# klausondrag/FOSVOS

Hardware: AMD Instinct MI355X
Metric: online fine-tune frames/sec (854x480) (higher is better)
Workload: dtype bf16; 1 GPU; OSVOS_VGG train_online one-shot fine-tune: 1x3x480x854 frame per step, fwd + class-balanced BCE + bwd, fused SGD step every 5 steps (BASELINE.json configs[1]); batch=1, avg_grad_every_n=5, activations=bf16 NHWC, fp32 accumulate, fp32 master weights, parallelism=single GPU

## Files before the change

fosvos_amd/csrc/common.hpp:

```cpp
#pragma once
#include <hip/hip_runtime.h>
#include <stdarg.h>
#include <algorithm>
#include <stdint.h>
#include <stdio.h>
#include <stdlib.h>
#include <string.h>

#include "../../include/fosvos_hip.h"

namespace fosvos {

extern thread_local char g_err[512];

inline int fail(int code, const char *fmt, ...) __attribute__((format(printf, 2, 3)));
inline int fail(int code, const char *fmt, ...) {
    va_list ap;
    va_start(ap, fmt);
    vsnprintf(g_err, sizeof(g_err), fmt, ap);
    va_end(ap);
    return code;
}

#define FOSVOS_HIP_CHECK(expr)                                                                         \
// ... 10 lines not shown
    } while (0)

#define FOSVOS_ENTER(device) FOSVOS_HIP_CHECK(hipSetDevice(device))
extern bool g_prof_on;
void prof_begin(const char *name, hipStream_t st, double flops);
void prof_end();
#define FOSVOS_PROF(name, st, flops)                                        \
    do {                                                                    \
        if (::fosvos::g_prof_on) ::fosvos::prof_begin(name, (hipStream_t)(st), flops); \
    } while (0)
#define FOSVOS_LAUNCH_CHECK()                            \
    do {                                                 \
        if (::fosvos::g_prof_on) ::fosvos::prof_end();   \
        FOSVOS_HIP_CHECK(hipGetLastError());             \
    } while (0)

struct WgradReduceEntry {
    const float *slabs;
    float *dw, *db;
    const float *bias_part;
    int64_t E_real, E_pad;
    int S, S_bias, Co, Cor, accumulate;
    int block_begin, n_blocks;
    int fold_begin, fold_blocks;
};
constexpr int kWgradReduceMax = 20;
struct WgradReduceTable {
    int n;
    WgradReduceEntry e[kWgradReduceMax];
};
int wgrad_impl(const uint16_t *x, const uint16_t *dy, float *dw, float *db, int N, int H, int W, int Ci, int Co,
               int accumulate, void *workspace, size_t workspace_bytes, int device, void *stream,
               WgradReduceTable *reduce, bool alone = false);
int first_wgrad_impl(const float *frame, const uint16_t *dy, float *dw, float *db, int N, int H, int W, int Co,
                     int accumulate, void *workspace, size_t workspace_bytes, int device, void *stream,
                     WgradReduceTable *reduce);
int wgrad_reduce_all(WgradReduceTable *reduce, int device, void *stream);
int wgrad_queue_reduce(const float *slabs, const float *bias_part, float *dw, float *db, int S, int S_bias, int64_t E_real,
                       int64_t E_pad, int Co, int Cor, int accumulate, WgradReduceTable *reduce, int device, void *stream);
struct HeadBwdArgs {
    const float *const *side;
    const int *hs, *ws;
    const float *const *filt, *const *filt1;
    const float *dsn_w, *fuse_w, *d_fused;
    const float *const *d_side_out;
    uint16_t *const *d_side;
    float *d_fuse_w, *d_fuse_b, *d_dsn_w, *d_dsn_b;
// ... 128 lines not shown
```

fosvos_amd/csrc/conv_wgrad.hip:

```cpp
#include <stdlib.h>

#include "common.hpp"

using namespace fosvos;

namespace {
constexpr int TH = 8;
constexpr int TPIX = TH * 16;
constexpr int HALO_W = 18;
constexpr int BCI = 64;

struct WgArgs {
    const uint16_t *x;
    const uint16_t *dy;
    float *slabs;
    float *bias_part;
    int N, H, W, Ci, Cy, Cor;
    int tiles_x, tiles_y, n_tiles, tiles_per_split;
    int lab;
    int S, n_ci, n_co, xcd_order;
};

typedef __attribute__((address_space(3))) s16x4 *lds_s16x4_ptr;

// ... 235 lines not shown
    const int ci = ci0 + wi * 16 + (lane & 15);
#pragma unroll
    for (int u = 0; u < NU; ++u)
#pragma unroll
        for (int r = 0; r < 4; ++r) {
            const int co = co0 + wc * 32 + u * 16 + 4 * g + r;
            if (co >= a.Cor || (a.lab & 1)) continue;
            float *d = slab + ((int64_t)co * a.Ci + ci) * 9;
#pragma unroll
            for (int t = 0; t < 9; ++t) d[t] = acc[t][u][r];
        }
#undef FOSVOS_W2_ROW
#undef FOSVOS_W2_PIECES_OF_ROW
#undef FOSVOS_W2_PIECE_ANY
#undef FOSVOS_W2_TILE_SCALARS
#undef FOSVOS_W2_ADVANCE
#undef FOSVOS_W2_STAGE
#undef FOSVOS_W2_PIECE_X
#undef FOSVOS_W2_PIECE_Y
}
}

constexpr int kFold = 8;

__global__ __launch_bounds__(256) void k_wgrad_fold(const WgradReduceTable t) {
    int e = 0;
    while (e + 1 < t.n && (int)blockIdx.x >= t.e[e + 1].fold_begin) ++e;
    const WgradReduceEntry &q = t.e[e];
    const int local = blockIdx.x - q.fold_begin;
    if (local >= q.fold_blocks) return;
    const int per_group = q.n_blocks;
    const int grp = local / per_group;
    const int64_t i4 = (int64_t)(local - grp * per_group) * 256 + threadIdx.x;
    if (i4 * 4 >= q.E_real) return;
    float *base = const_cast<float *>(q.slabs) + (int64_t)grp * kFold * q.E_pad + i4 * 4;
    const int n = min(kFold, q.S - grp * kFold);
    float4 v[kFold];
#pragma unroll
    for (int j = 0; j < kFold; ++j) v[j] = *reinterpret_cast<const float4 *>(base + (int64_t)min(j, n - 1) * q.E_pad);
    float4 acc = v[0];
#pragma unroll
    for (int j = 1; j < kFold; ++j)
        if (j < n) { acc.x += v[j].x; acc.y += v[j].y; acc.z += v[j].z; acc.w += v[j].w; }
    *reinterpret_cast<float4 *>(base) = acc;
}

__global__ __launch_bounds__(256) void k_wgrad_reduce(const WgradReduceTable t) {
    int e = 0;
    while (e + 1 < t.n && (int)blockIdx.x >= t.e[e + 1].block_begin) ++e;
    const WgradReduceEntry &q = t.e[e];
    const int local = blockIdx.x - q.block_begin;
    const int64_t i4 = (int64_t)local * 256 + threadIdx.x;
    const bool folded = q.fold_blocks > 0;
    const int n_src = folded ? (q.S + kFold - 1) / kFold : q.S;
    const int64_t stride = (folded ? kFold : 1) * q.E_pad;
    if (i4 * 4 < q.E_real) {
        const float *src = q.slabs + i4 * 4;
        float4 acc = make_float4(0.f, 0.f, 0.f, 0.f);
        for (int s0 = 0; s0 < n_src; s0 += 8) {
            float4 v[8];
#pragma unroll
            for (int j = 0; j < 8; ++j) v[j] = *reinterpret_cast<const float4 *>(src + (int64_t)min(s0 + j, n_src - 1) * stride);
#pragma unroll
            for (int j = 0; j < 8; ++j)
                if (s0 + j < n_src) { acc.x += v[j].x; acc.y += v[j].y; acc.z += v[j].z; acc.w += v[j].w; }
        }
        float4 *d = reinterpret_cast<float4 *>(q.dw + i4 * 4);
        if (q.accumulate) {
            const float4 o = *d;
            acc.x += o.x; acc.y += o.y; acc.z += o.z; acc.w += o.w;
        }
        *d = acc;
    }
    if (local == 0 && q.db) {
        __shared__ float s_part[256];
        int Cg = 1;
        while (Cg < q.Co && Cg < 256) Cg <<= 1;
        const int P = 256 / Cg, part = threadIdx.x / Cg, cl = threadIdx.x - part * Cg;
        const int per = (q.S_bias + P - 1) / P, s_lo = part * per, s_hi = min(s_lo + per, q.S_bias);
        for (int co0 = 0; co0 < q.Co; co0 += Cg) {
            const int co = co0 + cl;
            float acc_b = 0.f;
            if (co < q.Co) {
                for (int s0 = s_lo; s0 < s_hi; s0 += 16) {
                    float v[16];
#pragma unroll
                    for (int j = 0; j < 16; ++j) v[j] = q.bias_part[(int64_t)min(s0 + j, s_hi - 1) * q.Cor + co];
#pragma unroll
                    for (int j = 0; j < 16; ++j)
                        if (s0 + j < s_hi) acc_b += v[j];
                }
            }
            if (co0) __syncthreads();
            s_part[threadIdx.x] = acc_b;
            __syncthreads();
// ... 86 lines not shown
extern "C" int fosvos_conv3x3_wgrad_slabs(const uint16_t *x, const uint16_t *dy, int with_bias, int N, int H, int W, int Ci,
                                          int Co, void *workspace, size_t workspace_bytes, int device, void *stream) {
    WgradReduceTable sink;
    sink.n = 0;
    float dummy = 0.f;
    return fosvos::wgrad_impl(x, dy, &dummy, with_bias ? &dummy : nullptr, N, H, W, Ci, Co, 0, workspace, workspace_bytes,
                              device, stream, &sink);
}

int fosvos::wgrad_queue_reduce(const float *slabs, const float *bias_part, float *dw, float *db, int S, int S_bias,
                               int64_t E_real,
                               int64_t E_pad, int Co, int Cor, int accumulate, WgradReduceTable *reduce, int device,
                               void *stream) {
    WgradReduceTable local;
    local.n = 0;
    WgradReduceTable *t = reduce ? reduce : &local;
    FOSVOS_REQUIRE(t->n < kWgradReduceMax, FOSVOS_E_ARG, "wgrad: reduction queue full");
    FOSVOS_REQUIRE(E_real % 4 == 0 && E_pad % 4 == 0, FOSVOS_E_SHAPE, "wgrad: slab size must be a multiple of 4 floats");
    WgradReduceEntry &q = t->e[t->n];
    q.slabs = slabs; q.dw = dw; q.db = db; q.bias_part = db ? bias_part : nullptr;
    q.S = S; q.S_bias = S_bias; q.Co = Co; q.Cor = Cor; q.accumulate = accumulate;
    q.E_real = E_real;
    q.E_pad = E_pad;
    q.n_blocks = (int)cdiv(E_real / 4, 256);
    q.block_begin = t->n ? t->e[t->n - 1].block_begin + t->e[t->n - 1].n_blocks : 0;
    q.fold_blocks = S > kFold ? (int)cdiv(S, kFold) * q.n_blocks : 0;
    q.fold_begin = t->n ? t->e[t->n - 1].fold_begin + t->e[t->n - 1].fold_blocks : 0;
    ++t->n;
    return reduce ? FOSVOS_OK : fosvos::wgrad_reduce_all(t, device, stream);
}

int fosvos::wgrad_reduce_all(WgradReduceTable *reduce, int device, void *stream) {
    FOSVOS_REQUIRE(reduce, FOSVOS_E_ARG, "wgrad_reduce_all: null table");
    if (reduce->n == 0) return FOSVOS_OK;
    FOSVOS_ENTER(device);
    const WgradReduceEntry &last = reduce->e[reduce->n - 1];
    if (last.fold_begin + last.fold_blocks > 0) {
        FOSVOS_PROF("k_wgrad_fold", stream, 0.0);
        hipLaunchKernelGGL(k_wgrad_fold, dim3((unsigned)(last.fold_begin + last.fold_blocks)), dim3(256), 0,
                           (hipStream_t)stream, *reduce);
        FOSVOS_LAUNCH_CHECK();
    }
    FOSVOS_PROF("k_wgrad_reduce", stream, 0.0);
    hipLaunchKernelGGL(k_wgrad_reduce, dim3((unsigned)(last.block_begin + last.n_blocks)), dim3(256), 0, (hipStream_t)stream,
                       *reduce);
    FOSVOS_LAUNCH_CHECK();
    reduce->n = 0;
    return FOSVOS_OK;
}

int fosvos::wgrad_impl(const uint16_t *x, const uint16_t *dy, float *dw, float *db, int N, int H, int W, int Ci, int Co,
                       int accumulate, void *workspace, size_t workspace_bytes, int device, void *stream,
                       WgradReduceTable *reduce, bool alone) {
    FOSVOS_REQUIRE(x && dy && dw && workspace, FOSVOS_E_ARG, "conv3x3_wgrad: null pointer");
    if (int rc = check_shape(N, H, W, Ci, Co, "conv3x3_wgrad")) return rc;
    const Plan p = make_plan(N, H, W, Ci, Co, alone);
    FOSVOS_REQUIRE(workspace_bytes >= p.slab_bytes + p.bias_bytes, FOSVOS_E_WORKSPACE,
                   "conv3x3_wgrad: workspace %zu < %zu", workspace_bytes, p.slab_bytes + p.bias_bytes);
    FOSVOS_ENTER(device);
    hipStream_t st = (hipStream_t)stream;
    WgArgs a;
    a.x = x; a.dy = dy; a.slabs = reinterpret_cast<float *>(workspace);
    a.bias_part = db ? reinterpret_cast<float *>(reinterpret_cast<char *>(workspace) + p.slab_bytes) : nullptr;
    a.N = N; a.H = H; a.W = W; a.Ci = Ci; a.Cy = p.Cy; a.Cor = p.Cor;
    a.tiles_x = p.tiles_x; a.tiles_y = p.tiles_y; a.n_tiles = p.n_tiles; a.tiles_per_split = p.tps;
// ... 37 lines not shown
```

fosvos_amd/csrc/sgd.hip:

```cpp
#include "common.hpp"

using namespace fosvos;

namespace {
__global__ __launch_bounds__(256) void k_sgd(const fosvos_sgd_entry *__restrict__ table, float momentum,
                                              int flags) {
    const bool first_step = flags & FOSVOS_SGD_FIRST_STEP, zero = flags & FOSVOS_SGD_ZERO_GRAD;
    const fosvos_sgd_entry e = table[blockIdx.y];
    if (e.grad == nullptr || e.numel <= 0) return;
    float *__restrict__ p = e.param;
    float *__restrict__ g = const_cast<float *>(e.grad);
    float *__restrict__ m = e.momentum_buf;
    const float lr = e.lr, wd = e.weight_decay;
    const int64_t n = e.numel;
    const bool vec = (((uintptr_t)p | (uintptr_t)g | (uintptr_t)m) & 15) == 0;
    const int64_t n4 = vec ? (n >> 2) : 0;
    for (int64_t i = blockIdx.x * (int64_t)blockDim.x + threadIdx.x; i < n4; i += (int64_t)gridDim.x * blockDim.x) {
        float4 pv = reinterpret_cast<float4 *>(p)[i];
        const float4 gv = reinterpret_cast<const float4 *>(g)[i];
        float4 mv = first_step ? make_float4(0, 0, 0, 0) : reinterpret_cast<float4 *>(m)[i];
        float pp[4] = {pv.x, pv.y, pv.z, pv.w}, gg[4] = {gv.x, gv.y, gv.z, gv.w}, mm[4] = {mv.x, mv.y, mv.z, mv.w};
#pragma unroll
        for (int j = 0; j < 4; ++j) {
            const float d = wd != 0.f ? gg[j] + wd * pp[j] : gg[j];
            mm[j] = first_step ? d : momentum * mm[j] + d;
            pp[j] = pp[j] - lr * mm[j];
        }
        reinterpret_cast<float4 *>(p)[i] = make_float4(pp[0], pp[1], pp[2], pp[3]);
        reinterpret_cast<float4 *>(m)[i] = make_float4(mm[0], mm[1], mm[2], mm[3]);
        if (zero) reinterpret_cast<float4 *>(g)[i] = make_float4(0.f, 0.f, 0.f, 0.f);
    }
    for (int64_t i = n4 * 4 + blockIdx.x * (int64_t)blockDim.x + threadIdx.x; i < n;
         i += (int64_t)gridDim.x * blockDim.x) {
        const float d = wd != 0.f ? g[i] + wd * p[i] : g[i];
        const float mm = first_step ? d : momentum * m[i] + d;
        m[i] = mm;
        p[i] = p[i] - lr * mm;
        if (zero) g[i] = 0.f;
    }
}
}

extern "C" int fosvos_sgd_momentum_step(const fosvos_sgd_entry *table, int n_tensors, int64_t max_numel, float momentum,
                                        int first_step, int device, void *stream) {
    FOSVOS_REQUIRE(table, FOSVOS_E_ARG, "sgd_momentum_step: null table");
    FOSVOS_REQUIRE(n_tensors > 0 && n_tensors <= 65535 && max_numel > 0, FOSVOS_E_SHAPE,
                   "sgd_momentum_step: n_tensors=%d max_numel=%lld", n_tensors, (long long)max_numel);
    FOSVOS_ENTER(device);
    int64_t gx = cdiv(max_numel, 256 * 4);
    if (gx > 512) gx = 512;
    FOSVOS_PROF("k_sgd", stream, 0.0);
    hipLaunchKernelGGL(k_sgd, dim3((unsigned)gx, (unsigned)n_tensors), dim3(256), 0, (hipStream_t)stream, table,
                       momentum, first_step);
    FOSVOS_LAUNCH_CHECK();
    return FOSVOS_OK;
}
```

fosvos_amd/fosvos_hip/__init__.py:

```python
from __future__ import annotations

import ctypes
import os
import threading
from ctypes import POINTER, c_char_p, c_float, c_int, c_int64, c_size_t, c_uint, c_void_p

_HERE = os.path.dirname(os.path.abspath(__file__))
PKG_ROOT = os.path.dirname(_HERE)
LIB_PATH = os.environ.get("FOSVOS_HIP_LIB") or os.path.join(PKG_ROOT, "lib", "libfosvos_hip.so")
HEADER_PATH = os.path.join(os.path.dirname(PKG_ROOT), "include", "fosvos_hip.h")

ABI_VERSION = 27
CONV_RELU = 1
CONV_OUT_F32 = 2


class FosvosHipError(RuntimeError):
    pass


class SgdEntry(ctypes.Structure):
    _fields_ = [("param", c_void_p), ("grad", c_void_p), ("momentum_buf", c_void_p), ("numel", c_int64),
                ("lr", c_float), ("weight_decay", c_float)]


_P4 = c_void_p * 4
_I4 = c_int * 4
_P13 = c_void_p * 13


class VggWeights(ctypes.Structure):
    _fields_ = [("conv_w", _P13), ("conv_b", _P13), ("conv_wf", _P13), ("conv_wd", _P13),
                ("side_b", _P4), ("side_wf", _P4), ("side_wd", _P4), ("filt", _P4), ("filt1", _P4),
                ("dsn_w", c_void_p), ("dsn_b", c_void_p), ("fuse_w", c_void_p), ("fuse_b", c_void_p),
                ("filt_uniform", c_int)]


class VggGrads(ctypes.Structure):
    _fields_ = [("conv_w", _P13), ("conv_b", _P13), ("side_w", _P4), ("side_b", _P4),
                ("dsn_w", c_void_p), ("dsn_b", c_void_p), ("fuse_w", c_void_p), ("fuse_b", c_void_p),
                ("accumulate", c_int), ("defer_join", c_int), ("bucket_events", c_int), ("last_pass_of_cycle", c_int)]

_Z4 = c_size_t * 4
_Z13 = c_size_t * 13


# ... 88 lines not shown
    "fosvos_maxpool2x2_ceil_bwd": (c_int, [c_void_p, c_void_p, c_void_p, c_int, c_int, c_int, c_int, c_int, c_int,
                                           c_void_p]),
    "fosvos_head_fwd": (c_int, [POINTER(c_void_p), POINTER(c_int), POINTER(c_int), POINTER(c_void_p),
                                POINTER(c_void_p), c_void_p, c_void_p, c_void_p, c_void_p, c_void_p,
                                POINTER(c_void_p), c_int, c_int, c_int, c_int, c_int, c_void_p]),
    "fosvos_head_bwd": (c_int, [POINTER(c_void_p), POINTER(c_int), POINTER(c_int), POINTER(c_void_p),
                                POINTER(c_void_p), c_void_p, c_void_p, c_void_p, POINTER(c_void_p),
                                POINTER(c_void_p), c_void_p, c_void_p, c_void_p, c_void_p, c_int, c_int, c_int, c_int,
                                c_void_p, c_size_t, c_int, c_void_p]),
    "fosvos_head_bwd_workspace_bytes": (c_size_t, [c_int, c_int, c_int]),
    "fosvos_cbce_loss": (c_int, [c_void_p, c_void_p, c_int64, c_int, c_float, c_void_p, c_void_p, c_void_p, c_size_t,
                                 c_int, c_void_p]),
    "fosvos_cbce_workspace_bytes": (c_size_t, [c_int64]),
    "fosvos_cbce_loss_frames": (c_int, [c_void_p, c_void_p, c_int64, c_int, c_int, c_float, c_void_p, c_void_p, c_void_p,
                                        c_size_t, c_int, c_void_p]),
    "fosvos_cbce_loss_frames_parts": (c_int, [c_void_p, c_void_p, c_int64, c_int, c_int, c_float, c_void_p, c_void_p,
                                              c_void_p, c_size_t, c_int, c_int, c_void_p]),
    "fosvos_cbce_multi_workspace_bytes": (c_size_t, [c_int64, c_int, c_int]),
    "fosvos_cbce_loss_frames_multi": (c_int, [POINTER(c_void_p), c_void_p, c_int64, c_int, c_int, c_int, POINTER(c_float),
                                              c_void_p, POINTER(c_void_p), c_void_p, c_size_t, c_int, c_int, c_void_p]),
    "fosvos_cbce_loss_batch_counts": (c_int, [c_void_p, c_void_p, c_int64, c_int, c_float, c_void_p, c_void_p, c_void_p,
                                              c_void_p, c_size_t, c_int, c_void_p]),
    "fosvos_sgd_momentum_step": (c_int, [c_void_p, c_int, c_int64, c_float, c_int, c_int, c_void_p]),
    "fosvos_conv3x3_s2_fwd": (c_int, [c_void_p, c_void_p, c_void_p, c_void_p, c_int, c_int, c_int, c_int, c_int, c_uint,
                                      c_void_p, c_size_t, c_int, c_void_p]),
    "fosvos_conv3x3_fwd_add": (c_int, [c_void_p, c_void_p, c_void_p, c_void_p, c_void_p, c_int, c_int, c_int, c_int, c_int,
                                       c_uint, c_void_p, c_size_t, c_int, c_void_p]),
    "fosvos_fold_conv_bn": (c_int, [c_void_p, c_int, c_int, c_int, c_void_p, c_void_p, c_void_p, c_void_p, c_void_p,
                                    c_float, c_void_p, c_void_p, c_int, c_void_p]),
    "fosvos_conv2d_packed_dwords": (c_size_t, [c_int, c_int, c_int]),
    "fosvos_conv2d_bias_elems": (c_size_t, [c_int]),
    "fosvos_pack_conv2d_bn": (c_int, [c_void_p, c_int, c_int, c_int, c_void_p, c_void_p, c_void_p, c_void_p, c_void_p,
                                      c_float, c_void_p, c_void_p, c_int, c_void_p]),
    "fosvos_conv2d_plan": (c_int, [c_int, c_int, c_int, c_int, c_int, c_int, c_int, POINTER(Conv2dPlanInfo)]),
    "fosvos_conv2d_fwd": (c_int, [c_void_p, c_void_p, c_void_p, c_void_p, c_void_p, c_int, c_int, c_int, c_int, c_int,
                                  c_int, c_int, c_uint, c_int, c_void_p]),
    "fosvos_conv7x7_packed_elems": (c_size_t, [c_int]),
    "fosvos_pack_conv7x7_bn": (c_int, [c_void_p, c_int, c_void_p, c_void_p, c_void_p, c_void_p, c_float, c_void_p,
                                       c_void_p, c_int, c_void_p]),
    "fosvos_conv7x7s2_first_fwd": (c_int, [c_void_p, c_void_p, c_void_p, c_void_p, c_int, c_int, c_int, c_int, c_uint,
                                           c_int, c_void_p]),
    "fosvos_conv7x7s2_pool_first_fwd": (c_int, [c_void_p, c_void_p, c_void_p, c_void_p, c_int, c_int, c_int, c_int, c_int,
                                                c_void_p]),
    "fosvos_maxpool3x3s2_fwd": (c_int, [c_void_p, c_void_p, c_int, c_int, c_int, c_int, c_int, c_void_p]),
    "fosvos_deconv_head_fwd": (c_int, [POINTER(c_void_p), POINTER(c_int), POINTER(c_int), POINTER(c_int),
                                       POINTER(c_void_p), POINTER(c_void_p), c_void_p, c_void_p, c_void_p, c_void_p,
# ... 120 lines not shown
```

fosvos_amd/fosvos_hip/engine.py:

```python
from __future__ import annotations

import ctypes
import time
from dataclasses import dataclass
from typing import Dict, List, Optional, Sequence, Tuple

import torch

from . import Context, VggGrads, VggWeights, check, lib, ops, ptr_array4
from .options import EngineOptions, native_loop_from_env

STAGE_CHANNELS = ((64, 64), (128, 128), (256, 256, 256), (512, 512, 512), (512, 512, 512))
STAGE_IN = (3, 64, 128, 256, 512)
SIDE_CH = 16


def conv_module_index(stage: int, k: int) -> int:
    return 2 * k + (0 if stage == 0 else 1)


def param_names() -> List[str]:
    names = [f"upscale.{i}.weight" for i in range(4)] + [f"upscale_.{i}.weight" for i in range(4)]
    for s, chans in enumerate(STAGE_CHANNELS):
        for j in range(len(chans)):
            m = conv_module_index(s, j)
            names += [f"stages.{s}.{m}.weight", f"stages.{s}.{m}.bias"]
    for i in range(4):
        names += [f"side_prep.{i}.weight", f"side_prep.{i}.bias"]
    for i in range(4):
        names += [f"score_dsn.{i}.weight", f"score_dsn.{i}.bias"]
    names += ["fuse.weight", "fuse.bias"]
    return names


PARAM_NAMES = param_names()
PARAM_INDEX = {n: i for i, n in enumerate(PARAM_NAMES)}


@dataclass(slots=True)
class PassFlags:

    defer_wgrad_join: bool = False
    forward_one_stream: bool = False
    publish_grad_buckets: bool = False
    overwrite_grads: bool = False
    last_pass_of_cycle: bool = False


class PackedWeights:

    def __init__(self, options: Optional[EngineOptions] = None) -> None:
        self.options = options if options is not None else EngineOptions.from_env()
        self.flags = PassFlags()
        self._cache: Dict[str, Tuple[object, object, object]] = {}
        self._uniform: Dict[str, bool] = {}
        self.arenas = ArenaPool()

    @staticmethod
    def _key(t: torch.Tensor) -> Tuple[int, int]:
        return (t.data_ptr(), t._version)

    def invalidate(self) -> None:
        self._cache.clear()
        self._uniform.clear()

    def small(self, name: str, parts: Sequence[torch.Tensor]) -> torch.Tensor:
        key = tuple(self._key(t) for t in parts)
        hit = self._cache.get(name)
        if hit is not None and hit[0] == key:
            return hit[1]
        cat = torch.cat([t.detach().reshape(-1) for t in parts]).contiguous()
        self._cache[name] = (key, cat, tuple(t.untyped_storage() for t in parts))
        return cat

    def conv(self, name: str, w: torch.Tensor):
        key = self._key(w)
        hit = self._cache.get(name)
        if hit is not None and hit[0] == key:
            return hit[1]
        packed = ops.pack_conv3x3_weights(w.detach(), True, True)
        self._cache[name] = (key, packed, w.untyped_storage())
        return packed

    def conv_many(self, named: Sequence[Tuple[str, torch.Tensor]]):
        stale = []
        for name, w in named:
            hit = self._cache.get(name)
            if hit is None or hit[0] != self._key(w):
                stale.append((name, w))
        if stale:
            packed = ops.pack_conv3x3_weights_multi([w.detach() for _, w in stale])
            for (name, w), pk in zip(stale, packed):
                self._cache[name] = (self._key(w), pk, w.untyped_storage())
        return [self._cache[name][1] for name, _ in named]

    def deconv_diag(self, name: str, w: torch.Tensor) -> torch.Tensor:
        key = self._key(w)
        hit = self._cache.get(name)
        if hit is not None and hit[0] == key:
            return hit[1]
        wd = w.detach()
        c = wd.shape[0]
        idx = torch.arange(c, device=wd.device)
        diag = wd[idx, idx]
        if c > 1:
            off = torch.count_nonzero(wd) - torch.count_nonzero(diag)
            if int(off) != 0:
                raise NotImplementedError(
                    f"{name}: transposed-conv weight has off-diagonal (cross-channel) entries; the HIP head "
                    f"implements the per-channel (diagonal) form the reference initialises and freezes")
        diag = diag.permute(1, 2, 0).contiguous()
        self._cache[name] = (key, diag, w.untyped_storage())
        self._uniform[name] = bool((diag == diag[..., :1]).all().item())
        return diag

    def head_uniform_mask(self, P: Dict[str, torch.Tensor]) -> int:
# ... 485 lines not shown
```

fosvos_amd/fosvos_hip/sgd.py:

```python
from __future__ import annotations

import ctypes

import torch
from torch import optim

from . import SgdEntry, check, lib


class FusedSGD(optim.SGD):
    def __init__(self, params, lr=1e-3, momentum=0, dampening=0, weight_decay=0, nesterov=False, **kw):
        if dampening != 0 or nesterov:
            raise NotImplementedError("FusedSGD implements the reference recipe: dampening=0, nesterov=False")
        kw.pop("foreach", None)
        kw.pop("fused", None)
        super().__init__(params, lr=lr, momentum=momentum, dampening=dampening, weight_decay=weight_decay,
                         nesterov=nesterov, **kw)
        self._tables = {}

    @torch.no_grad()
    def step(self, closure=None, only=None, tag="all", zero_grad=False):
        only_ids = None if only is None else {id(p) for p in only}
        loss = None
        if closure is not None:
            with torch.enable_grad():
                loss = closure()
        entries = []
        momentum = None
        device = None
        max_numel = 0
        keep_alive = []
        zero_after = []
        updated = []
        for group in self.param_groups:
            if group.get("dampening", 0) != 0 or group.get("nesterov", False):
                raise NotImplementedError("FusedSGD: dampening/nesterov are not implemented")
            m = float(group["momentum"])
            if momentum is None:
                momentum = m
            elif m != momentum:
                raise NotImplementedError("FusedSGD: one momentum value for all groups (as in the reference recipe)")
            for p in group["params"]:
                if p.grad is None or (only_ids is not None and id(p) not in only_ids):
                    continue
                if not p.is_cuda:
                    raise RuntimeError("FusedSGD: parameters must live on the GPU (no CPU fallback)")
                if p.dtype != torch.float32 or not p.is_contiguous():
                    raise TypeError("FusedSGD: fp32 contiguous parameters only")
                g = p.grad
                if g.dtype != torch.float32 or not g.is_contiguous():
                    g = g.contiguous().float()
                    keep_alive.append(g)
                    if zero_grad:
                        zero_after.append(p.grad)
                st = self.state[p]
                buf = st.get("momentum_buffer")
                if buf is None:
                    buf = torch.zeros_like(p, memory_format=torch.contiguous_format)
                    st["momentum_buffer"] = buf
                device = p.device
                entries.append((p.data_ptr(), g.data_ptr(), buf.data_ptr(), p.numel(), float(group["lr"]),
                                float(group["weight_decay"])))
                if float(group["lr"]) != 0.0:
                    updated.append(p)
                max_numel = max(max_numel, p.numel())
        if not entries:
            return loss
        n = len(entries)
        nbytes = n * ctypes.sizeof(SgdEntry)
        tab = self._tables.setdefault(tag, {"entries": None, "host": None, "dev": None, "event": None})
        if entries != tab["entries"]:
            if tab["host"] is None or tab["host"].numel() < nbytes:
                tab["host"] = torch.empty(max(nbytes, 4096), dtype=torch.uint8).pin_memory()
                tab["dev"] = torch.empty(max(nbytes, 4096), dtype=torch.uint8, device=device)
            if tab["event"] is not None:
                tab["event"].synchronize()
            arr = (SgdEntry * n).from_address(tab["host"].data_ptr())
            for i, e in enumerate(entries):
                arr[i].param, arr[i].grad, arr[i].momentum_buf, arr[i].numel, arr[i].lr, arr[i].weight_decay = e
            tab["dev"][:nbytes].copy_(tab["host"][:nbytes], non_blocking=True)
            tab["event"] = torch.cuda.Event()
            tab["event"].record()
            tab["entries"] = entries
        idx = device.index if device.index is not None else torch.cuda.current_device()
        check(lib().fosvos_sgd_momentum_step(tab["dev"].data_ptr(), n, max_numel, momentum, 2 if zero_grad else 0, idx,
                                             torch.cuda.current_stream(idx).cuda_stream), "sgd_momentum_step")
        for p in updated:
            torch.autograd.graph.increment_version(p)
        for g in zero_after:
            g.zero_()
        del keep_alive
        return loss
```

include/fosvos_hip.h:

```cpp
#ifndef FOSVOS_HIP_H
#define FOSVOS_HIP_H

#include <stddef.h>
#include <stdint.h>

#ifdef __cplusplus
extern "C" {
#endif

#define FOSVOS_ABI_VERSION 27

#define FOSVOS_OK 0
#define FOSVOS_E_SHAPE (-1)
#define FOSVOS_E_ARG (-2)
#define FOSVOS_E_WORKSPACE (-3)
#define FOSVOS_E_HIP (-4)

#define FOSVOS_CONV_RELU 1u
#define FOSVOS_CONV_OUT_F32 2u
#define FOSVOS_CONV_FP32_MATH 4u

int fosvos_abi_version(void);

typedef struct fosvos_profile_record {
    char name[96];
    int launches;
    double ms;
    double flops;
} fosvos_profile_record;
int fosvos_profile_start(int device, int max_launches);
int fosvos_profile_stop(int device, fosvos_profile_record *out, int capacity, int *n_out);
const char *fosvos_last_error(void);
const char *fosvos_build_arch(void);
// ... 111 lines not shown
                                  int size_average, float grad_scale, float *loss_out, float *grad, void *workspace,
                                  size_t workspace_bytes, int parts, int device, void *stream);
#define FOSVOS_CBCE_MAX_MAPS 8
size_t fosvos_cbce_multi_workspace_bytes(int64_t frame_numel, int n_frames, int n_maps);
int fosvos_cbce_loss_frames_multi(const float *const *logits, const float *label, int64_t frame_numel, int n_frames,
                                  int n_maps, int size_average, const float *map_scale, float *loss_out, float *const *grad,
                                  void *workspace, size_t workspace_bytes, int parts, int device, void *stream);
int fosvos_cbce_loss_batch_counts(const float *logits, const float *label, int64_t numel, int size_average,
                                  float grad_scale, const double *batch_counts, float *loss_out, float *grad,
                                  void *workspace, size_t workspace_bytes, int device, void *stream);

#define FOSVOS_SGD_FIRST_STEP 1
#define FOSVOS_SGD_ZERO_GRAD 2
typedef struct fosvos_sgd_entry {
    float *param;
    const float *grad;
    float *momentum_buf;
    int64_t numel;
    float lr;
    float weight_decay;
} fosvos_sgd_entry;
int fosvos_sgd_momentum_step(const fosvos_sgd_entry *table, int n_tensors, int64_t max_numel, float momentum,
                             int first_step, int device, void *stream);

int fosvos_augment_sample(const uint8_t *frame, const uint8_t *mask, int H, int W, int flip, const int32_t *col_taps,
                          const float *col_w, const int32_t *row_taps, const float *row_w, const int32_t *col_near,
                          const int32_t *row_near, int OH, int OW, const float *img_lut, const float *gt_lut, float *image,
                          float *gt, int device, void *stream);

int fosvos_prob_bytes(const float *logits, int N, int H, int W, float *minmax, uint8_t *out, int device, void *stream);
size_t fosvos_jf_workspace_bytes(int N, int H, int W);
int fosvos_jf_counts(const float *logits, const uint8_t *gt, int N, int H, int W, int radius, int32_t *counts,
                     void *workspace, size_t workspace_bytes, int device, void *stream);

size_t fosvos_png_capacity_bytes(int N, int H, int W);
size_t fosvos_png_workspace_bytes(int N, int H, int W);
int fosvos_png_encode(const uint8_t *bytes, int N, int H, int W, uint8_t *out, size_t capacity, int32_t *lengths,
                      void *workspace, size_t workspace_bytes, int device, void *stream);

size_t fosvos_png_workspace_bytes_mode(int N, int H, int W, int huffman);
int fosvos_png_encode_mode(const uint8_t *bytes, int N, int H, int W, int huffman, uint8_t *out, size_t capacity,
                           int32_t *lengths, void *workspace, size_t workspace_bytes, int device, void *stream);

size_t fosvos_jpeg_capacity_bytes(int N, int H, int W, int components);
size_t fosvos_jpeg_workspace_bytes(int N, int H, int W, int components);
int fosvos_jpeg_encode(const uint8_t *frames, int N, int H, int W, int components, int quality, uint8_t *out,
// ... 122 lines not shown
```

Baseline: 1265 frames/s.

## Fuse conv weight repacking into SGD step and merge wgrad fold into reduce

```diff
diff --git a/fosvos_amd/csrc/common.hpp b/fosvos_amd/csrc/common.hpp
--- a/fosvos_amd/csrc/common.hpp
+++ b/fosvos_amd/csrc/common.hpp
@@ -56,7 +56,7 @@
     int64_t E_real, E_pad;
     int S, S_bias, Co, Cor, accumulate;
     int block_begin, n_blocks;
-    int fold_begin, fold_blocks;
+    int cols;
 };
 constexpr int kWgradReduceMax = 20;
 struct WgradReduceTable {
diff --git a/fosvos_amd/csrc/conv_wgrad.hip b/fosvos_amd/csrc/conv_wgrad.hip
--- a/fosvos_amd/csrc/conv_wgrad.hip
+++ b/fosvos_amd/csrc/conv_wgrad.hip
@@ -281,55 +281,75 @@
 }
 
 constexpr int kFold = 8;
-
-__global__ __launch_bounds__(256) void k_wgrad_fold(const WgradReduceTable t) {
-    int e = 0;
-    while (e + 1 < t.n && (int)blockIdx.x >= t.e[e + 1].fold_begin) ++e;
-    const WgradReduceEntry &q = t.e[e];
-    const int local = blockIdx.x - q.fold_begin;
-    if (local >= q.fold_blocks) return;
-    const int per_group = q.n_blocks;
-    const int grp = local / per_group;
-    const int64_t i4 = (int64_t)(local - grp * per_group) * 256 + threadIdx.x;
-    if (i4 * 4 >= q.E_real) return;
-    float *base = const_cast<float *>(q.slabs) + (int64_t)grp * kFold * q.E_pad + i4 * 4;
-    const int n = min(kFold, q.S - grp * kFold);
-    float4 v[kFold];
-#pragma unroll
-    for (int j = 0; j < kFold; ++j) v[j] = *reinterpret_cast<const float4 *>(base + (int64_t)min(j, n - 1) * q.E_pad);
-    float4 acc = v[0];
-#pragma unroll
-    for (int j = 1; j < kFold; ++j)
-        if (j < n) { acc.x += v[j].x; acc.y += v[j].y; acc.z += v[j].z; acc.w += v[j].w; }
-    *reinterpret_cast<float4 *>(base) = acc;
+constexpr int kReduceDirect = 256;
+
+int reduce_cols(int S) {
+    if (S <= kFold) return kReduceDirect;
+    const int G = (S + kFold - 1) / kFold;
+    int gt = 4;
+    while (gt < G && gt < 32) gt <<= 1;
+    return 256 / gt;
 }
 
 __global__ __launch_bounds__(256) void k_wgrad_reduce(const WgradReduceTable t) {
+    __shared__ float s_grp[256 * 4];
     int e = 0;
     while (e + 1 < t.n && (int)blockIdx.x >= t.e[e + 1].block_begin) ++e;
     const WgradReduceEntry &q = t.e[e];
     const int local = blockIdx.x - q.block_begin;
-    const int64_t i4 = (int64_t)local * 256 + threadIdx.x;
-    const bool folded = q.fold_blocks > 0;
-    const int n_src = folded ? (q.S + kFold - 1) / kFold : q.S;
-    const int64_t stride = (folded ? kFold : 1) * q.E_pad;
-    if (i4 * 4 < q.E_real) {
-        const float *src = q.slabs + i4 * 4;
-        float4 acc = make_float4(0.f, 0.f, 0.f, 0.f);
-        for (int s0 = 0; s0 < n_src; s0 += 8) {
-            float4 v[8];
-#pragma unroll
-            for (int j = 0; j < 8; ++j) v[j] = *reinterpret_cast<const float4 *>(src + (int64_t)min(s0 + j, n_src - 1) * stride);
-#pragma unroll
-            for (int j = 0; j < 8; ++j)
-                if (s0 + j < n_src) { acc.x += v[j].x; acc.y += v[j].y; acc.z += v[j].z; acc.w += v[j].w; }
-        }
-        float4 *d = reinterpret_cast<float4 *>(q.dw + i4 * 4);
-        if (q.accumulate) {
-            const float4 o = *d;
-            acc.x += o.x; acc.y += o.y; acc.z += o.z; acc.w += o.w;
-        }
-        *d = acc;
+    if (q.cols == kReduceDirect) {
+        const int64_t i4 = (int64_t)local * 256 + threadIdx.x;
+        if (i4 * 4 < q.E_real) {
+            const float *src = q.slabs + i4 * 4;
+            float4 acc = make_float4(0.f, 0.f, 0.f, 0.f);
+            for (int s0 = 0; s0 < q.S; s0 += 8) {
+                float4 v[8];
+#pragma unroll
+                for (int j = 0; j < 8; ++j) v[j] = *reinterpret_cast<const float4 *>(src + (int64_t)min(s0 + j, q.S - 1) * q.E_pad);
+#pragma unroll
+                for (int j = 0; j < 8; ++j)
+                    if (s0 + j < q.S) { acc.x += v[j].x; acc.y += v[j].y; acc.z += v[j].z; acc.w += v[j].w; }
+            }
+            float4 *d = reinterpret_cast<float4 *>(q.dw + i4 * 4);
+            if (q.accumulate) {
+                const float4 o = *d;
+                acc.x += o.x; acc.y += o.y; acc.z += o.z; acc.w += o.w;
+            }
+            *d = acc;
+        }
+    } else {
+        const int C = q.cols, GT = 256 / C;
+        const int col = threadIdx.x & (C - 1), gt = threadIdx.x / C;
+        const int64_t i4 = (int64_t)local * C + col;
+        const bool live = i4 * 4 < q.E_real;
+        const int G = (q.S + kFold - 1) / kFold;
+        float tot = 0.f;
+        for (int g0 = 0; g0 < G; g0 += GT) {
+            const int grp = g0 + gt;
+            if (live && grp < G) {
+                const float *base = q.slabs + (int64_t)grp * kFold * q.E_pad + i4 * 4;
+                const int n = min(kFold, q.S - grp * kFold);
+                float4 v[kFold];
+#pragma unroll
+                for (int j = 0; j < kFold; ++j) v[j] = *reinterpret_cast<const float4 *>(base + (int64_t)min(j, n - 1) * q.E_pad);
+                float4 acc = v[0];
+#pragma unroll
+                for (int j = 1; j < kFold; ++j)
+                    if (j < n) { acc.x += v[j].x; acc.y += v[j].y; acc.z += v[j].z; acc.w += v[j].w; }
+                *reinterpret_cast<float4 *>(s_grp + (gt * C + col) * 4) = acc;
+            }
+            __syncthreads();
+            if ((int)threadIdx.x < 4 * C) {
+                const int ng = min(GT, G - g0);
+                for (int j = 0; j < ng; ++j) tot += s_grp[j * C * 4 + threadIdx.x];
+            }
+            __syncthreads();
+        }
+        const int64_t f = (int64_t)local * C * 4 + threadIdx.x;
+        if ((int)threadIdx.x < 4 * C && f < q.E_real) {
+            if (q.accumulate) tot += q.dw[f];
+            q.dw[f] = tot;
+        }
     }
     if (local == 0 && q.db) {
         __shared__ float s_part[256];
@@ -462,10 +482,9 @@
     q.S = S; q.S_bias = S_bias; q.Co = Co; q.Cor = Cor; q.accumulate = accumulate;
     q.E_real = E_real;
     q.E_pad = E_pad;
-    q.n_blocks = (int)cdiv(E_real / 4, 256);
+    q.cols = reduce_cols(S);
+    q.n_blocks = (int)cdiv(E_real / 4, q.cols);
     q.block_begin = t->n ? t->e[t->n - 1].block_begin + t->e[t->n - 1].n_blocks : 0;
-    q.fold_blocks = S > kFold ? (int)cdiv(S, kFold) * q.n_blocks : 0;
-    q.fold_begin = t->n ? t->e[t->n - 1].fold_begin + t->e[t->n - 1].fold_blocks : 0;
     ++t->n;
     return reduce ? FOSVOS_OK : fosvos::wgrad_reduce_all(t, device, stream);
 }
@@ -475,12 +494,6 @@
     if (reduce->n == 0) return FOSVOS_OK;
     FOSVOS_ENTER(device);
     const WgradReduceEntry &last = reduce->e[reduce->n - 1];
-    if (last.fold_begin + last.fold_blocks > 0) {
-        FOSVOS_PROF("k_wgrad_fold", stream, 0.0);
-        hipLaunchKernelGGL(k_wgrad_fold, dim3((unsigned)(last.fold_begin + last.fold_blocks)), dim3(256), 0,
-                           (hipStream_t)stream, *reduce);
-        FOSVOS_LAUNCH_CHECK();
-    }
     FOSVOS_PROF("k_wgrad_reduce", stream, 0.0);
     hipLaunchKernelGGL(k_wgrad_reduce, dim3((unsigned)(last.block_begin + last.n_blocks)), dim3(256), 0, (hipStream_t)stream,
                        *reduce);
diff --git a/fosvos_amd/csrc/sgd.hip b/fosvos_amd/csrc/sgd.hip
--- a/fosvos_amd/csrc/sgd.hip
+++ b/fosvos_amd/csrc/sgd.hip
@@ -3,11 +3,14 @@
 using namespace fosvos;
 
 namespace {
-__global__ __launch_bounds__(256) void k_sgd(const fosvos_sgd_entry *__restrict__ table, float momentum,
-                                              int flags) {
-    const bool first_step = flags & FOSVOS_SGD_FIRST_STEP, zero = flags & FOSVOS_SGD_ZERO_GRAD;
-    const fosvos_sgd_entry e = table[blockIdx.y];
-    if (e.grad == nullptr || e.numel <= 0) return;
+__device__ __forceinline__ void sgd_update(float &p, float g, float &m, float lr, float wd, float momentum, bool first_step) {
+    const float d = wd != 0.f ? g + wd * p : g;
+    m = first_step ? d : momentum * m + d;
+    p = p - lr * m;
+}
+
+template <class E>
+__device__ __forceinline__ void sgd_elementwise(const E &e, float momentum, bool first_step, bool zero) {
     float *__restrict__ p = e.param;
     float *__restrict__ g = const_cast<float *>(e.grad);
     float *__restrict__ m = e.momentum_buf;
@@ -21,22 +24,107 @@
         float4 mv = first_step ? make_float4(0, 0, 0, 0) : reinterpret_cast<float4 *>(m)[i];
         float pp[4] = {pv.x, pv.y, pv.z, pv.w}, gg[4] = {gv.x, gv.y, gv.z, gv.w}, mm[4] = {mv.x, mv.y, mv.z, mv.w};
 #pragma unroll
-        for (int j = 0; j < 4; ++j) {
-            const float d = wd != 0.f ? gg[j] + wd * pp[j] : gg[j];
-            mm[j] = first_step ? d : momentum * mm[j] + d;
-            pp[j] = pp[j] - lr * mm[j];
-        }
+        for (int j = 0; j < 4; ++j) sgd_update(pp[j], gg[j], mm[j], lr, wd, momentum, first_step);
         reinterpret_cast<float4 *>(p)[i] = make_float4(pp[0], pp[1], pp[2], pp[3]);
         reinterpret_cast<float4 *>(m)[i] = make_float4(mm[0], mm[1], mm[2], mm[3]);
         if (zero) reinterpret_cast<float4 *>(g)[i] = make_float4(0.f, 0.f, 0.f, 0.f);
     }
     for (int64_t i = n4 * 4 + blockIdx.x * (int64_t)blockDim.x + threadIdx.x; i < n;
          i += (int64_t)gridDim.x * blockDim.x) {
-        const float d = wd != 0.f ? g[i] + wd * p[i] : g[i];
-        const float mm = first_step ? d : momentum * m[i] + d;
+        float pp = p[i], mm = first_step ? 0.f : m[i];
+        sgd_update(pp, g[i], mm, lr, wd, momentum, first_step);
         m[i] = mm;
-        p[i] = p[i] - lr * mm;
+        p[i] = pp;
         if (zero) g[i] = 0.f;
+    }
+}
+
+__global__ __launch_bounds__(256) void k_sgd(const fosvos_sgd_entry *__restrict__ table, float momentum,
+                                              int flags) {
+    const fosvos_sgd_entry e = table[blockIdx.y];
+    if (e.grad == nullptr || e.numel <= 0) return;
+    sgd_elementwise(e, momentum, flags & FOSVOS_SGD_FIRST_STEP, flags & FOSVOS_SGD_ZERO_GRAD);
+}
+
+__global__ __launch_bounds__(256) void k_sgd_pack(const fosvos_sgd_pack_entry *__restrict__ table, float momentum, int flags,
+                                                   int co_t) {
+    __shared__ float tile[32][289];
+    const bool first_step = flags & FOSVOS_SGD_FIRST_STEP, zero = flags & FOSVOS_SGD_ZERO_GRAD;
+    const fosvos_sgd_pack_entry e = table[blockIdx.y];
+    if (e.grad == nullptr || e.numel <= 0) return;
+    if (e.w_fwd == nullptr && e.w_dgrad == nullptr) {
+        sgd_elementwise(e, momentum, first_step, zero);
+        return;
+    }
+    float *__restrict__ p = e.param;
+    float *__restrict__ g = const_cast<float *>(e.grad);
+    float *__restrict__ m = e.momentum_buf;
+    const float lr = e.lr, wd = e.weight_decay;
+    const int Co = e.Co, Ci = e.Ci, nkb = Ci / 32;
+    const int n_tiles = (Co + 31) / 32 * 32 / co_t * nkb;
+    const int co_pad = (Co + 15) / 16 * 16, ci_pad = (Ci + 15) / 16 * 16;
+    const bool vec = (((uintptr_t)p | (uintptr_t)g | (uintptr_t)m) & 15) == 0;
+    for (int t = blockIdx.x; t < n_tiles; t += gridDim.x) {
+        const int cb = t / nkb, kb = t - cb * nkb;
+        const int co0 = cb * co_t, ci0 = kb * 32;
+        if (vec) {
+            for (int i = threadIdx.x; i < co_t * 72; i += 256) {
+                const int r = i / 72, c = (i - r * 72) * 4;
+                float pp[4] = {0.f, 0.f, 0.f, 0.f};
+                if (co0 + r < Co) {
+                    const int64_t at = ((int64_t)(co0 + r) * Ci + ci0) * 9 + c;
+                    const float4 pv = *reinterpret_cast<const float4 *>(p + at), gv = *reinterpret_cast<const float4 *>(g + at);
+                    const float4 mv = first_step ? make_float4(0, 0, 0, 0) : *reinterpret_cast<const float4 *>(m + at);
+                    float gg[4] = {gv.x, gv.y, gv.z, gv.w}, mm[4] = {mv.x, mv.y, mv.z, mv.w};
+                    pp[0] = pv.x; pp[1] = pv.y; pp[2] = pv.z; pp[3] = pv.w;
+#pragma unroll
+                    for (int j = 0; j < 4; ++j) sgd_update(pp[j], gg[j], mm[j], lr, wd, momentum, first_step);
+                    *reinterpret_cast<float4 *>(p + at) = make_float4(pp[0], pp[1], pp[2], pp[3]);
+                    *reinterpret_cast<float4 *>(m + at) = make_float4(mm[0], mm[1], mm[2], mm[3]);
+                    if (zero) *reinterpret_cast<float4 *>(g + at) = make_float4(0.f, 0.f, 0.f, 0.f);
+                }
+                tile[r][c] = pp[0]; tile[r][c + 1] = pp[1]; tile[r][c + 2] = pp[2]; tile[r][c + 3] = pp[3];
+            }
+        } else {
+            for (int i = threadIdx.x; i < co_t * 288; i += 256) {
+                const int r = i / 288, c = i - r * 288;
+                float pp = 0.f;
+                if (co0 + r < Co) {
+                    const int64_t at = ((int64_t)(co0 + r) * Ci + ci0) * 9 + c;
+                    float mm = first_step ? 0.f : m[at];
+                    pp = p[at];
+                    sgd_update(pp, g[at], mm, lr, wd, momentum, first_step);
+                    p[at] = pp;
+                    m[at] = mm;
+                    if (zero) g[at] = 0.f;
+                }
+                tile[r][c] = pp;
+            }
+        }
+        __syncthreads();
+        if (e.w_fwd) {
+            for (int q = threadIdx.x; q < 9 * 4 * co_t; q += 256) {
+                const int l = q % co_t, kc = (q / co_t) & 3, tap = q / (4 * co_t);
+                if (co0 + l >= co_pad) continue;
+                float f[8];
+#pragma unroll
+                for (int j = 0; j < 8; ++j) f[j] = tile[l][(kc * 8 + j) * 9 + tap];
+                *reinterpret_cast<uint4 *>(e.w_fwd + ((((int64_t)kb * 9 + tap) * 4 + kc) * co_pad + co0 + l) * 8) = pack8(f);
+            }
+        }
+        if (e.w_dgrad) {
+            const int n_kc = co_t / 8;
+            for (int q = threadIdx.x; q < 9 * n_kc * 32; q += 256) {
+                const int l = q & 31, kc = (q >> 5) % n_kc, tap = (q >> 5) / n_kc;
+                float f[8];
+#pragma unroll
+                for (int j = 0; j < 8; ++j) f[j] = tile[kc * 8 + j][l * 9 + tap];
+                const int co = co0 + kc * 8;
+                *reinterpret_cast<uint4 *>(e.w_dgrad + ((((int64_t)(co >> 5) * 9 + (8 - tap)) * 4 + ((co >> 3) & 3)) * ci_pad + ci0 + l) * 8) =
+                    pack8(f);
+            }
+        }
+        __syncthreads();
     }
 }
 }
@@ -55,3 +143,22 @@
     FOSVOS_LAUNCH_CHECK();
     return FOSVOS_OK;
 }
+
+extern "C" int fosvos_sgd_momentum_step_pack(const fosvos_sgd_pack_entry *table, int n_tensors, int64_t max_numel,
+                                             int pack_tiles, int max_pack_tiles, float momentum, int flags, int device,
+                                             void *stream) {
+    FOSVOS_REQUIRE(table, FOSVOS_E_ARG, "sgd_momentum_step_pack: null table");
+    FOSVOS_REQUIRE(n_tensors > 0 && n_tensors <= 65535 && max_numel > 0, FOSVOS_E_SHAPE,
+                   "sgd_momentum_step_pack: n_tensors=%d max_numel=%lld", n_tensors, (long long)max_numel);
+    FOSVOS_REQUIRE(pack_tiles >= 0 && max_pack_tiles >= 0 && max_pack_tiles <= pack_tiles, FOSVOS_E_ARG,
+                   "sgd_momentum_step_pack: pack_tiles=%d max_pack_tiles=%d", pack_tiles, max_pack_tiles);
+    FOSVOS_ENTER(device);
+    const int co_t = pack_tiles < 256 ? 8 : 32;
+    int64_t gx = std::max<int64_t>(cdiv(max_numel, 256 * 4), (int64_t)max_pack_tiles * (32 / co_t));
+    if (gx > 512) gx = 512;
+    FOSVOS_PROF(pack_tiles ? "k_sgd_pack" : "k_sgd", stream, 0.0);
+    hipLaunchKernelGGL(k_sgd_pack, dim3((unsigned)gx, (unsigned)n_tensors), dim3(256), 0, (hipStream_t)stream, table, momentum,
+                       flags, co_t);
+    FOSVOS_LAUNCH_CHECK();
+    return FOSVOS_OK;
+}
diff --git a/fosvos_amd/fosvos_hip/__init__.py b/fosvos_amd/fosvos_hip/__init__.py
--- a/fosvos_amd/fosvos_hip/__init__.py
+++ b/fosvos_amd/fosvos_hip/__init__.py
@@ -10,7 +10,7 @@
 LIB_PATH = os.environ.get("FOSVOS_HIP_LIB") or os.path.join(PKG_ROOT, "lib", "libfosvos_hip.so")
 HEADER_PATH = os.path.join(os.path.dirname(PKG_ROOT), "include", "fosvos_hip.h")
 
-ABI_VERSION = 27
+ABI_VERSION = 28
 CONV_RELU = 1
 CONV_OUT_F32 = 2
 
@@ -22,6 +22,12 @@
 class SgdEntry(ctypes.Structure):
     _fields_ = [("param", c_void_p), ("grad", c_void_p), ("momentum_buf", c_void_p), ("numel", c_int64),
                 ("lr", c_float), ("weight_decay", c_float)]
+
+
+class SgdPackEntry(ctypes.Structure):
+    _fields_ = [("param", c_void_p), ("grad", c_void_p), ("momentum_buf", c_void_p), ("numel", c_int64),
+                ("lr", c_float), ("weight_decay", c_float), ("w_fwd", c_void_p), ("w_dgrad", c_void_p), ("Co", c_int),
+                ("Ci", c_int)]
 
 
 _P4 = c_void_p * 4
@@ -156,6 +162,7 @@
     "fosvos_cbce_loss_batch_counts": (c_int, [c_void_p, c_void_p, c_int64, c_int, c_float, c_void_p, c_void_p, c_void_p,
                                               c_void_p, c_size_t, c_int, c_void_p]),
     "fosvos_sgd_momentum_step": (c_int, [c_void_p, c_int, c_int64, c_float, c_int, c_int, c_void_p]),
+    "fosvos_sgd_momentum_step_pack": (c_int, [c_void_p, c_int, c_int64, c_int, c_int, c_float, c_int, c_int, c_void_p]),
     "fosvos_conv3x3_s2_fwd": (c_int, [c_void_p, c_void_p, c_void_p, c_void_p, c_int, c_int, c_int, c_int, c_int, c_uint,
                                       c_void_p, c_size_t, c_int, c_void_p]),
     "fosvos_conv3x3_fwd_add": (c_int, [c_void_p, c_void_p, c_void_p, c_void_p, c_void_p, c_int, c_int, c_int, c_int, c_int,
diff --git a/fosvos_amd/fosvos_hip/engine.py b/fosvos_amd/fosvos_hip/engine.py
--- a/fosvos_amd/fosvos_hip/engine.py
+++ b/fosvos_amd/fosvos_hip/engine.py
@@ -2,6 +2,7 @@
 
 import ctypes
 import time
+import weakref
 from dataclasses import dataclass
 from typing import Dict, List, Optional, Sequence, Tuple
 
@@ -47,6 +48,17 @@
     last_pass_of_cycle: bool = False
 
 
+_LIVE_CACHES: "weakref.WeakSet[PackedWeights]" = weakref.WeakSet()
+
+
+def step_image_slot(w: torch.Tensor):
+    for packs in _LIVE_CACHES:
+        hit = packs.step_images(w)
+        if hit is not None:
+            return packs, hit[0], hit[1]
+    return None
+
+
 class PackedWeights:
 
     def __init__(self, options: Optional[EngineOptions] = None) -> None:
@@ -54,7 +66,9 @@
         self.flags = PassFlags()
         self._cache: Dict[str, Tuple[object, object, object]] = {}
         self._uniform: Dict[str, bool] = {}
+        self._conv_by_ptr: Dict[int, str] = {}
         self.arenas = ArenaPool()
+        _LIVE_CACHES.add(self)
 
     @staticmethod
     def _key(t: torch.Tensor) -> Tuple[int, int]:
@@ -63,6 +77,23 @@
     def invalidate(self) -> None:
         self._cache.clear()
         self._uniform.clear()
+        self._conv_by_ptr.clear()
+
+    def _put_conv(self, name: str, w: torch.Tensor, packed) -> None:
+        self._cache[name] = (self._key(w), packed, w.untyped_storage())
+        self._conv_by_ptr[w.data_ptr()] = name
+
+    def step_images(self, w: torch.Tensor):
+        name = self._conv_by_ptr.get(w.data_ptr())
+        hit = self._cache.get(name) if name is not None else None
+        if hit is None or hit[0][0] != w.data_ptr() or not isinstance(hit[1], tuple) or hit[1][0] is None or hit[1][1] is None:
+            return None
+        return name, hit[1]
+
+    def adopt(self, name: str, w: torch.Tensor, images) -> None:
+        hit = self._cache.get(name)
+        if hit is not None and hit[1] is images:
+            self._cache[name] = (self._key(w), images, hit[2])
 
     def small(self, name: str, parts: Sequence[torch.Tensor]) -> torch.Tensor:
         key = tuple(self._key(t) for t in parts)
@@ -79,7 +110,7 @@
         if hit is not None and hit[0] == key:
             return hit[1]
         packed = ops.pack_conv3x3_weights(w.detach(), True, True)
-        self._cache[name] = (key, packed, w.untyped_storage())
+        self._put_conv(name, w, packed)
         return packed
 
     def conv_many(self, named: Sequence[Tuple[str, torch.Tensor]]):
@@ -91,7 +122,7 @@
         if stale:
             packed = ops.pack_conv3x3_weights_multi([w.detach() for _, w in stale])
             for (name, w), pk in zip(stale, packed):
-                self._cache[name] = (self._key(w), pk, w.untyped_storage())
+                self._put_conv(name, w, pk)
         return [self._cache[name][1] for name, _ in named]
 
     def deconv_diag(self, name: str, w: torch.Tensor) -> torch.Tensor:
diff --git a/fosvos_amd/fosvos_hip/sgd.py b/fosvos_amd/fosvos_hip/sgd.py
--- a/fosvos_amd/fosvos_hip/sgd.py
+++ b/fosvos_amd/fosvos_hip/sgd.py
@@ -5,7 +5,7 @@
 import torch
 from torch import optim
 
-from . import SgdEntry, check, lib
+from . import SgdPackEntry, check, lib
 
 
 class FusedSGD(optim.SGD):
@@ -20,6 +20,7 @@
 
     @torch.no_grad()
     def step(self, closure=None, only=None, tag="all", zero_grad=False):
+        from . import engine
         only_ids = None if only is None else {id(p) for p in only}
         loss = None
         if closure is not None:
@@ -32,6 +33,8 @@
         keep_alive = []
         zero_after = []
         updated = []
+        adopted = []
+        pack_tiles = max_pack_tiles = 0
         for group in self.param_groups:
             if group.get("dampening", 0) != 0 or group.get("nesterov", False):
                 raise NotImplementedError("FusedSGD: dampening/nesterov are not implemented")
@@ -59,15 +62,30 @@
                     buf = torch.zeros_like(p, memory_format=torch.contiguous_format)
                     st["momentum_buffer"] = buf
                 device = p.device
+                wf = wd = co = ci = 0
+                if p.dim() == 4 and p.shape[2:] == (3, 3) and p.shape[1] % 32 == 0:
+                    slot = engine.step_image_slot(p)
+                    co, ci = int(p.shape[0]), int(p.shape[1])
+                    if slot is not None and (slot[2][0].numel() != ci * 9 * ((co + 15) // 16 * 16)
+                                             or slot[2][1].numel() != (co + 31) // 32 * 32 * 9 * ((ci + 15) // 16 * 16)):
+                        slot = None
+                    if slot is None:
+                        co = ci = 0
+                    else:
+                        wf, wd = slot[2][0].data_ptr(), slot[2][1].data_ptr()
+                        tiles = (co + 31) // 32 * (ci // 32)
+                        pack_tiles += tiles
+                        max_pack_tiles = max(max_pack_tiles, tiles)
+                        adopted.append((slot[0], slot[1], slot[2], p))
                 entries.append((p.data_ptr(), g.data_ptr(), buf.data_ptr(), p.numel(), float(group["lr"]),
-                                float(group["weight_decay"])))
+                                float(group["weight_decay"]), wf, wd, co, ci))
                 if float(group["lr"]) != 0.0:
                     updated.append(p)
                 max_numel = max(max_numel, p.numel())
         if not entries:
             return loss
         n = len(entries)
-        nbytes = n * ctypes.sizeof(SgdEntry)
+        nbytes = n * ctypes.sizeof(SgdPackEntry)
         tab = self._tables.setdefault(tag, {"entries": None, "host": None, "dev": None, "event": None})
         if entries != tab["entries"]:
             if tab["host"] is None or tab["host"].numel() < nbytes:
@@ -75,18 +93,23 @@
                 tab["dev"] = torch.empty(max(nbytes, 4096), dtype=torch.uint8, device=device)
             if tab["event"] is not None:
                 tab["event"].synchronize()
-            arr = (SgdEntry * n).from_address(tab["host"].data_ptr())
+            arr = (SgdPackEntry * n).from_address(tab["host"].data_ptr())
             for i, e in enumerate(entries):
-                arr[i].param, arr[i].grad, arr[i].momentum_buf, arr[i].numel, arr[i].lr, arr[i].weight_decay = e
+                (arr[i].param, arr[i].grad, arr[i].momentum_buf, arr[i].numel, arr[i].lr, arr[i].weight_decay, wf, wd,
+                 arr[i].Co, arr[i].Ci) = e
+                arr[i].w_fwd, arr[i].w_dgrad = wf or None, wd or None
             tab["dev"][:nbytes].copy_(tab["host"][:nbytes], non_blocking=True)
             tab["event"] = torch.cuda.Event()
             tab["event"].record()
             tab["entries"] = entries
         idx = device.index if device.index is not None else torch.cuda.current_device()
-        check(lib().fosvos_sgd_momentum_step(tab["dev"].data_ptr(), n, max_numel, momentum, 2 if zero_grad else 0, idx,
-                                             torch.cuda.current_stream(idx).cuda_stream), "sgd_momentum_step")
+        check(lib().fosvos_sgd_momentum_step_pack(tab["dev"].data_ptr(), n, max_numel, pack_tiles, max_pack_tiles, momentum,
+                                                  2 if zero_grad else 0, idx, torch.cuda.current_stream(idx).cuda_stream),
+              "sgd_momentum_step_pack")
         for p in updated:
             torch.autograd.graph.increment_version(p)
+        for packs, name, images, p in adopted:
+            packs.adopt(name, p, images)
         for g in zero_after:
             g.zero_()
         del keep_alive
diff --git a/include/fosvos_hip.h b/include/fosvos_hip.h
--- a/include/fosvos_hip.h
+++ b/include/fosvos_hip.h
@@ -8,7 +8,7 @@
 extern "C" {
 #endif
 
-#define FOSVOS_ABI_VERSION 27
+#define FOSVOS_ABI_VERSION 28
 
 #define FOSVOS_OK 0
 #define FOSVOS_E_SHAPE (-1)
@@ -166,6 +166,18 @@
 } fosvos_sgd_entry;
 int fosvos_sgd_momentum_step(const fosvos_sgd_entry *table, int n_tensors, int64_t max_numel, float momentum,
                              int first_step, int device, void *stream);
+typedef struct fosvos_sgd_pack_entry {
+    float *param;
+    const float *grad;
+    float *momentum_buf;
+    int64_t numel;
+    float lr;
+    float weight_decay;
+    uint16_t *w_fwd, *w_dgrad;
+    int Co, Ci;
+} fosvos_sgd_pack_entry;
+int fosvos_sgd_momentum_step_pack(const fosvos_sgd_pack_entry *table, int n_tensors, int64_t max_numel, int pack_tiles,
+                                  int max_pack_tiles, float momentum, int flags, int device, void *stream);
 
 int fosvos_augment_sample(const uint8_t *frame, const uint8_t *mask, int H, int W, int flip, const int32_t *col_taps,
                           const float *col_w, const int32_t *row_taps, const float *row_w, const int32_t *col_near,
```

New measurement: 1275 frames/s (median of 6 runs). Within noise of the previous version (+0.8%).
